# tkmct/halo2-aes

Hardware: AMD Instinct MI355X
Metric: AES-128 block witnesses/sec (higher is better)
Workload: dtype u8

## Files before the change

### halo2-aes_amd/_build.py

```python
from __future__ import annotations

import os
import shutil
import subprocess
from pathlib import Path

PKG = Path(__file__).resolve().parent
ROOT = PKG.parent
CSRC = PKG / "csrc"
LIB = PKG / "libaesw.so"
HOST_LIB = PKG / "libaesw_host.so"
INCLUDE = ROOT / "include"


def _newer(target: Path, sources) -> bool:
    if not target.exists():
        return False
    t = target.stat().st_mtime
    return all(Path(s).stat().st_mtime <= t for s in sources)


def _run(cmd, cwd=None):
    proc = subprocess.run(cmd, cwd=cwd, stdout=subprocess.PIPE, stderr=subprocess.STDOUT, text=True)
    if proc.returncode != 0:
# ... 6 lines not shown
        if cand and Path(cand).exists():
            return cand
    raise RuntimeError("hipcc not found")


def _build(target: Path, deps, command, force: bool, in_place: bool = False) -> Path:
    if not force and _newer(target, deps):
        return target
    import fcntl
    with open(PKG / ".build.lock", "w") as lock:
        fcntl.flock(lock, fcntl.LOCK_EX)
        try:
            if not force and _newer(target, deps):
                return target
            tmp = target if in_place else target.with_suffix(".so.tmp%d" % os.getpid())
            _run(command(tmp))
            os.replace(tmp, target)
        finally:
            fcntl.flock(lock, fcntl.LOCK_UN)
    return target


def build_host(force: bool = False) -> Path:
    host = PKG / "host"
    srcs = [host / "host_capi.cpp"]
    deps = srcs + [INCLUDE / "aesw.h", INCLUDE / "aesw_host.h", host / "halo2_lite.hpp", host / "aes_gadget.hpp", LIB]
    return _build(HOST_LIB, deps, lambda tmp: ["g++", "-O2", "-std=c++17", "-fPIC", "-shared", "-Wall", "-o", str(tmp)] + [str(s) for s in srcs] +
                  ["-L" + str(PKG), "-laesw", "-Wl,-rpath,$ORIGIN"], force)


PRODUCT_SOURCES = [CSRC / n for n in ("aesw_kernels.hip", "aesw_api.cpp", "aesw_keyring.cpp", "aesw_hostpath.cpp", "aesw_arena.cpp",
                                      "aesw_comm.cpp", "aesw_group.cpp", "aesw_circuits.cpp")]
PRODUCT_HEADERS = [CSRC / n for n in ("aesw_lane.h", "aesw_layout.h", "aesw_flush.h", "aesw_slabmap.h", "aesw_check.h", "aesw_check_dev.h", "aesw_internal.h", "aesw_ctx.h",
                                      "aesw_keyring.h", "aesw_options.h", "aesw_placement.h")] + \
    [INCLUDE / "aesw.h"]


def _hipcc_shared(sources, out, extra_flags=(), link=()):
    return [hipcc_path(), "--offload-arch=gfx950", "-O3", "-std=c++17", "-fPIC", "-shared", "-Wall", "-pthread"] + list(extra_flags) + \
        ["-o", str(out)] + [str(s) for s in sources] + list(link)


def build_product(force: bool = False, extra_flags=(), out: Path = LIB, extra_sources=()) -> Path:
    srcs = PRODUCT_SOURCES + [Path(s) for s in extra_sources]
    return _build(Path(out), srcs + PRODUCT_HEADERS, lambda tmp: _hipcc_shared(srcs, tmp, extra_flags), force)


SATELLITE_HEADERS = [CSRC / n for n in ("aesw_check_dev.h", "aesw_check.h", "aesw_layout.h", "aesw_slabmap.h", "aesw_internal.h", "aesw_ctx.h",
                                        "aesw_keyring.h", "aesw_options.h", "aesw_placement.h")] + [INCLUDE / "aesw.h"]
SATELLITES = {
    "circ": ([CSRC / "circ" / "aesw_circ_check.hip"], [CSRC / "aesw_circ_search.h"], INCLUDE / "aesw_circ.h"),
    "cols": ([CSRC / "cols" / "aesw_cols_check.hip"], [CSRC / "aesw_circ_search.h"], INCLUDE / "aesw_cols.h"),
    "vals": ([CSRC / "vals" / "aesw_vals_check.hip"], [CSRC / "aesw_vals_check.h"], INCLUDE / "aesw_vals.h"),
    "acc": ([CSRC / "acc" / "aesw_acc.hip"], [CSRC / "aesw_mult.h", CSRC / "aesw_mult_dev.h", CSRC / "aesw_run.h", INCLUDE / "aesw_mult.h"], INCLUDE / "aesw_acc.h"),
    "perm": ([CSRC / "perm" / "aesw_perm.hip"], [CSRC / "aesw_mult.h", CSRC / "aesw_perm.h", INCLUDE / "aesw_mult.h"], INCLUDE / "aesw_perm.h"),
    "vacc": ([CSRC / "vacc" / "aesw_vacc.hip"], [CSRC / "aesw_mult.h", CSRC / "aesw_mult_dev.h", CSRC / "aesw_run.h", CSRC / "aesw_vals_check.h", CSRC / "aesw_vacc.h",
              INCLUDE / "aesw_mult.h"],
             INCLUDE / "aesw_vacc.h"),
    "mult": ([CSRC / "mult" / "aesw_mult.hip"], [CSRC / "aesw_mult.h", CSRC / "aesw_mult_dev.h"], INCLUDE / "aesw_mult.h"),
}
CIRC_LIB, COLS_LIB, VALS_LIB, ACC_LIB, PERM_LIB, VACC_LIB, MULT_LIB = (PKG / ("libaesw_%s.so" % name) for name in SATELLITES)

FIELD_LIBRARIES = {
    "theta": ([CSRC / "theta" / "aesw_theta.hip"], [CSRC / "aesw_fr.h", CSRC / "aesw_theta.h", CSRC / "aesw_mult.h", INCLUDE / "aesw_mult.h"],
              INCLUDE / "aesw_theta.h"),
}
THETA_LIB = PKG / "libaesw_theta.so"
# ... 7 lines not shown
```

### halo2-aes_amd/api.py

```python
from __future__ import annotations

import ctypes as C
from collections import namedtuple
from pathlib import Path

import numpy as np

from . import constants as K

_PKG = Path(__file__).resolve().parent
LIB_PATH = _PKG / "libaesw.so"
HOST_LIB_PATH = _PKG / "libaesw_host.so"
COLS_LIB_PATH = _PKG / "libaesw_cols.so"
VALS_LIB_PATH = _PKG / "libaesw_vals.so"
MULT_LIB_PATH = _PKG / "libaesw_mult.so"
ACC_LIB_PATH = _PKG / "libaesw_acc.so"
VACC_LIB_PATH = _PKG / "libaesw_vacc.so"
PERM_LIB_PATH = _PKG / "libaesw_perm.so"
THETA_LIB_PATH = _PKG / "libaesw_theta.so"
CIRC_LIB_PATH = _PKG / "libaesw_circ.so"

STATUS = {
    0: "AESW_OK", 1: "AESW_ERR_INVALID_ARG", 2: "AESW_ERR_NO_DEVICE", 3: "AESW_ERR_HIP", 4: "AESW_ERR_NOMEM",
    5: "AESW_ERR_CAPACITY", 6: "AESW_ERR_NO_KEY", 7: "AESW_ERR_MISMATCH", 8: "AESW_ERR_UNSATISFIED", 9: "AESW_ERR_COMM",
# ... 601 lines not shown
        ct = torch.empty((n, 16), dtype=torch.uint8, device=dev) if want_ct else None
        key = None
        if key_slab:
            m = n if n_keys is None else n_keys
            key = KeyWitness(torch.empty(m * K.WORDS_ROWS, dtype=torch.uint8, device=dev),
                             *[torch.empty(m * key_column_stride(layout, c), dtype=torch.uint8, device=dev)
                               for c in range(3)], None)
        return Witness(cols[0], cols[1], cols[2], ct, key)

    def alloc_columns(self, n: int, layout: int = K.LAYOUT_PACKED, want_ct: bool = False, key_slab: bool = False, key_only: bool = False):
        torch = self._torch()
        cols = Columns()
        if key_only:
            key_slab = True
        self._check(self._lib.aesw_columns_alloc(self._h, n, layout, 2 if key_only else (1 if key_slab else 0), 1 if want_ct else 0, C.byref(cols)),
                    "aesw_columns_alloc")
        dev = self._dev()

        def view(ptr, nbytes):
            if not ptr or not nbytes:
                return torch.empty(0, dtype=torch.uint8, device=dev)
            return torch.as_tensor(_DevView(ptr, nbytes), device=dev)

        x, y, z = (view(getattr(cols, c), n * column_stride(layout, i) if not key_only else 0) for i, c in enumerate("xyz"))
        ct = view(cols.ct, n * 16).view(n, 16) if want_ct else None
        key = None
        if key_slab:
            key = KeyWitness(view(cols.key.w, n * K.WORDS_ROWS), *[view(getattr(cols.key, c), n * key_column_stride(layout, i))
                                                                   for i, c in enumerate(("kx", "ky", "kz"))], None)
        wit = ArenaWitness(x, y, z, ct, key)
        wit.columns = cols
        self._arenas[id(cols)] = cols
        self.last_arena = {"candidates": int(cols.candidates), "chosen": int(cols.chosen), "probe_us": float(cols.probe_us),
                           "fill_us": float(cols.fill_us), "bytes": int(cols.bytes)}
        return wit

    def free_columns(self, wit) -> None:
        cols = getattr(wit, "columns", None)
        if cols is None or self._arenas.pop(id(cols), None) is None:
            raise ValueError("not a witness of alloc_columns (or already freed)")
        wit.columns = None
        self._check(self._lib.aesw_columns_free(self._h, C.byref(cols)), "aesw_columns_free")

    def schedule_key(self, key, layout: int = K.LAYOUT_PACKED, key_slab: bool = True):
        torch = self._torch()
        key = self._u8(key, "key")
        if key.numel() != 16:
            raise ValueError("key must be uint8[16]")
        out = ks = None
        if key_slab:
            dev = self._dev()
            out = KeyWitness(torch.empty(K.WORDS_ROWS, dtype=torch.uint8, device=dev),
                             *[torch.empty(key_column_stride(layout, c), dtype=torch.uint8, device=dev) for c in range(3)],
                             None)
            ks = KeySlab(*[t.data_ptr() for t in out[:4]])
        rc = self._lib.aesw_schedule_key_device(self._h, key.data_ptr(), layout, _ptr(ks),
                                                self._stream())
        self._check(rc, "aesw_schedule_key_device")
        return out

    def encrypt_witness(self, pt, keys, layout: int = K.LAYOUT_PACKED, out: Witness | None = None,
                        want_ct: bool = False, key_slab: bool = False) -> Witness:
        pt = self._u8(pt, "pt")
        if pt.dim() != 2 or pt.shape[1] != 16:
            raise ValueError("pt must be [n,16]")
        n = pt.shape[0]
        if keys is None:
# ... 804 lines not shown
```

### halo2-aes_amd/csrc/aesw_api.cpp

```cpp
#include <hip/hip_runtime.h>

#include <cstdio>
#include <cstdlib>
#include <cstring>
#include <algorithm>
#include <mutex>
#include <new>
#include <string>
#include <vector>

#include "../../include/aesw.h"
#include "aesw_internal.h"
#include "aesw_check.h"

using namespace aesw;

#include "aesw_ctx.h"

namespace {

bool aligned16(const void *p) { return (reinterpret_cast<uintptr_t>(p) & 15u) == 0; }
bool aligned4(const void *p) { return (reinterpret_cast<uintptr_t>(p) & 3u) == 0; }
bool valid_layout(int l) { return aesw_valid_layout(l); }

// ... 84 lines not shown
    return AESW_OK;
}

int check_witness_impl(aesw_ctx *ctx, const uint8_t *d_pt, const uint8_t *d_keys, int per_block_keys, uint64_t n, int layout,
                       const uint8_t *d_x, const uint8_t *d_y, const uint8_t *d_z, const uint8_t *d_ct, const aesw_key_slab *ks,
                       aesw_check_report *d_report, void *stream, bool skip_shared_key) {
    static_assert(sizeof(aesw_check_report) == 7 * sizeof(uint64_t), "the kernels address the report as seven u64");
    if (!ctx || !d_report || (layout != AESW_LAYOUT_DENSE && layout != AESW_LAYOUT_PACKED)) return AESW_ERR_INVALID_ARG;
    if (per_block_keys && n && !d_keys) return AESW_ERR_INVALID_ARG;
    if (n && (!d_pt || !d_x || !d_y || !d_z || !ks || !ks->w || !ks->kx || !ks->ky || !ks->kz)) return AESW_ERR_INVALID_ARG;
    if (n && (!aligned4(d_pt) || !aligned4(d_x) || !aligned4(d_y) || !aligned4(d_z) || !aligned4(ks->w) || !aligned4(ks->kx) || !aligned4(ks->ky) ||
              !aligned4(ks->kz) || (reinterpret_cast<uintptr_t>(d_report) & 7u)))
        return AESW_ERR_INVALID_ARG;
    DeviceGuard g(ctx->device);
    if (!g.ok) return AESW_ERR_NO_DEVICE;
    const int li = layout == AESW_LAYOUT_DENSE ? 0 : 1;
    const CheckGeo cg = check_geo(layout);
    CheckParams p{};
    p.pt = d_pt; p.keys = d_keys; p.x = d_x; p.y = d_y; p.z = d_z; p.ct = d_ct;
    if (ks) set_key_slab(p, ks);
    p.table = ctx->d_chktab[li];
    p.tab768 = ctx->d_tables;
    p.report = reinterpret_cast<uint64_t *>(d_report);
    p.n = n;
    p.per_block_keys = per_block_keys ? 1u : 0u;
    p.skip_shared_key = skip_shared_key ? 1u : 0u;
    set_strides(p, slab_strides(layout));
    p.bi = cg.bi;
    p.img = (cg.bi + cg.ki + 15u) & ~15u;
    HIP_TRY(ctx, launch_check(p, reinterpret_cast<hipStream_t>(stream)));
    return AESW_OK;
}

namespace {

struct EncLaunch {
    const uint8_t *d_pt, *d_keys;
    int per_block_keys;
    uint64_t n;
    int layout;
    uint8_t *d_x, *d_y, *d_z, *d_ct;
    KeyOut ko;
    bool kemit;
};

bool validate_encrypt(const aesw_ctx *ctx, const uint8_t *d_pt, const uint8_t *d_keys, int per_block_keys, uint64_t n, int layout, uint8_t *d_x,
                     uint8_t *d_y, uint8_t *d_z, uint8_t *d_ct, const aesw_key_slab *ks, EncLaunch *L, int *status) {
    *status = AESW_ERR_INVALID_ARG;
    if (!ctx || !valid_layout(layout)) return false;
    if (!d_keys) {
        if (per_block_keys) return false;
        if (!ctx->keys.has_key()) { *status = AESW_ERR_NO_KEY; return false; }
    }
    *L = EncLaunch{d_pt, d_keys, per_block_keys, n, layout, d_x, d_y, d_z, d_ct, KeyOut{nullptr, nullptr, nullptr, nullptr}, false};
    *status = AESW_OK;
    if (n == 0) return false;
    *status = AESW_ERR_INVALID_ARG;
    const bool has_x = slab_strides(layout).x != 0;
    if (!d_pt || (has_x && !d_x) || !d_y || !d_z) return false;
    if ((has_x && !aligned16(d_x)) || !aligned16(d_y) || !aligned16(d_z) || !aligned4(d_pt) || (d_keys && !aligned4(d_keys)) ||
        (d_ct && !aligned4(d_ct)))
        return false;
    if (!key_out_of(ks, &L->ko)) return false;
    L->kemit = L->ko.w || L->ko.kx || L->ko.ky || L->ko.kz;
    if (!d_keys && L->kemit) return false;
    *status = AESW_OK;
    return true;
}

int enqueue_encrypt(aesw_ctx *ctx, const EncLaunch &L, hipStream_t s) {
    if (!L.per_block_keys && L.kemit) {
        KeyParams kp{L.d_keys, ctx->d_tables, L.ko, nullptr, 1, 0, 0};
        HIP_TRY(ctx, launch_key(kp, L.layout, ctx->xt, 1, ctx->opt.key_nt, 0u, s));
    }
    const int km = L.per_block_keys ? 0 : (L.d_keys ? 1 : 2);
    KeyRing::Access rd;
    if (km == 2) {
        const int rc = ctx->keys.begin_read(ctx, s, &rd);
        if (rc != AESW_OK) return rc;
    }
    EncParams p{L.d_pt, L.d_keys, reinterpret_cast<const uint32_t *>(rd.d), ctx->d_tables, ctx->d_ftab[L.layout], L.d_x, L.d_y, L.d_z, L.d_ct,
                L.per_block_keys ? L.ko : KeyOut{nullptr, nullptr, nullptr, nullptr}, L.n, 0, 0};
#ifdef AESW_TRACE
    p.trace = ctx->trace;
#endif
    HIP_TRY(ctx, launch_encrypt(p, L.layout, ctx->xt, km, L.per_block_keys && L.kemit, auto_waves(ctx, L.layout, L.per_block_keys != 0),
                                ctx->opt.nt, (uint32_t)ctx->opt.grid_cap, ctx->opt.xcd_remap, (uint32_t)ctx->opt.lds_pad, s));
    return km == 2 ? ctx->keys.end_read(ctx, rd) : AESW_OK;
}

template <class Issue>
int fork_join(aesw_ctx *ctx, hipStream_t s, uint32_t ns, uint32_t count, Issue &&issue) {
    if (!ctx->ev_fork) HIP_TRY(ctx, hipEventCreateWithFlags(&ctx->ev_fork, hipEventDisableTiming));
    for (uint32_t j = 0; j < ns; ++j) {
        if (!ctx->s_batch[j]) HIP_TRY(ctx, hipStreamCreateWithFlags(&ctx->s_batch[j], hipStreamNonBlocking));
        if (!ctx->ev_join[j]) HIP_TRY(ctx, hipEventCreateWithFlags(&ctx->ev_join[j], hipEventDisableTiming));
    }
    HIP_TRY(ctx, hipEventRecord(ctx->ev_fork, s));
    for (uint32_t j = 0; j < ns; ++j) HIP_TRY(ctx, hipStreamWaitEvent(ctx->s_batch[j], ctx->ev_fork, 0));
    int rc = AESW_OK;
    for (uint32_t i = 0; i < count && rc == AESW_OK; ++i) rc = issue(i, ctx->s_batch[i % ns]);
    for (uint32_t j = 0; j < ns; ++j) {
        const hipError_t e1 = hipEventRecord(ctx->ev_join[j], ctx->s_batch[j]);
        const hipError_t e2 = e1 == hipSuccess ? hipStreamWaitEvent(s, ctx->ev_join[j], 0) : e1;
        if (e2 != hipSuccess && rc == AESW_OK) rc = fail_hip(ctx, e2, "join of the batch streams");
    }
    return rc;
}

int encrypt_lone(aesw_ctx *ctx, const EncLaunch &L, hipStream_t s) {
    if (ctx->opt.split_small <= 1 || L.per_block_keys || L.kemit || L.n < ((uint64_t)1 << 15) || L.n > ((uint64_t)1 << 17)) return enqueue_encrypt(ctx, L, s);
    const uint32_t parts = (uint32_t)ctx->opt.split_small;
    const uint64_t per = ((L.n + parts - 1) / parts + 47) / 48 * 48;
    const uint32_t cnt = (uint32_t)((L.n + per - 1) / per);
    const SlabStrides st = slab_strides(L.layout);
    return fork_join(ctx, s, cnt, cnt, [&](uint32_t i, hipStream_t si) {
        const uint64_t lo = i * per;
        EncLaunch part = L;
        part.d_pt += lo * 16;
        part.n = L.n - lo < per ? L.n - lo : per;
// ... 395 lines not shown
```

### halo2-aes_amd/csrc/aesw_arena.cpp

```cpp
#include <hip/hip_runtime.h>

#include <algorithm>
#include <chrono>
#include <cstring>
#include <vector>

#include "../../include/aesw.h"
#include "aesw_ctx.h"
#include "aesw_internal.h"

using namespace aesw;

namespace {
bool valid_layout(int l) { return aesw_valid_layout(l); }
}

extern "C" {

namespace {

int vmm_build(aesw_ctx *ctx, size_t total, size_t chunk, void **out) {
    hipMemAllocationProp prop = {};
    prop.type = hipMemAllocationTypePinned;
    prop.location.type = hipMemLocationTypeDevice;
    prop.location.id = ctx->device;
    hipMemAccessDesc acc = {};
    acc.location = prop.location;
    acc.flags = hipMemAccessFlagsProtReadWrite;
    void *va = nullptr;
    HIP_TRY(ctx, hipMemAddressReserve(&va, total, 0, nullptr, 0));
    size_t mapped = 0;
    hipError_t e = hipSuccess;
    while (mapped < total && e == hipSuccess) {
        const size_t sz = total - mapped < chunk ? total - mapped : chunk;
        hipMemGenericAllocationHandle_t h;
        e = hipMemCreate(&h, sz, &prop, 0);
        if (e != hipSuccess) break;
        e = hipMemMap(reinterpret_cast<uint8_t *>(va) + mapped, sz, 0, h, 0);
        (void)hipMemRelease(h);
        if (e == hipSuccess) mapped += sz;
// ... 55 lines not shown
    DeviceGuard g(ctx->device);
    if (!g.ok) return AESW_ERR_NO_DEVICE;
    auto fill_out = [&](uint8_t *b) {
        auto at = [&](int i) -> uint8_t * { return size[i] ? b + off[i] : nullptr; };
        out->x = at(0); out->y = at(1); out->z = at(2); out->ct = at(3);
        out->key.w = at(4); out->key.kx = at(5); out->key.ky = at(6); out->key.kz = at(7);
    };
    int probe = ctx->opt.arena_probe < 0 ? (n >= ((uint64_t)1 << 16) ? 8 : 0) : ctx->opt.arena_probe;
    if (probe == 0) {
        uint8_t *raw = nullptr;
        HIP_TRY(ctx, hipMalloc(reinterpret_cast<void **>(&raw), end + align));
        out->base = raw;
        out->bytes = end + align;
        fill_out(raw + (align - reinterpret_cast<uintptr_t>(raw) % align) % align);
        return AESW_OK;
    }
    if (ctx->opt.arena_cache_on) {
        for (size_t i = ctx->arena_cache.size(); i-- > 0;) {
            aesw_ctx::ArenaRec &c = ctx->arena_cache[i];
            if (c.n == n && c.layout == layout && c.with_key_slab == with_key_slab && c.with_ct == (with_ct ? 1 : 0) && c.xcd == ctx->opt.xcd_remap) {
                *out = c.cols;
                out->candidates = 0;
                ctx->vmm_arenas.push_back(std::move(c));
                ctx->arena_cache.erase(ctx->arena_cache.begin() + (long)i);
                ++ctx->arena_cache_hits;
                return AESW_OK;
            }
        }
        size_t free_b = 0, total_b = 0;
        if (hipMemGetInfo(&free_b, &total_b) != hipSuccess) { (void)hipGetLastError(); free_b = 0; }
        if (free_b < 2 * end + ((size_t)16 << 30)) cache_trim(ctx, 0);
    }
    const auto t_search = std::chrono::steady_clock::now();
    auto over_budget = [&]() {
        if (ctx->opt.arena_probe_budget_ms <= 0) return false;
        return std::chrono::duration_cast<std::chrono::milliseconds>(std::chrono::steady_clock::now() - t_search).count() > ctx->opt.arena_probe_budget_ms;
    };
    using Range = aesw_ctx::ArenaRange;
    const size_t MiB2 = (size_t)2 << 20;
    auto round2m = [&](uint64_t v) { return (size_t)((v + MiB2 - 1) / MiB2 * MiB2); };
    auto build = [&](int kind, size_t bytes, Range *r) -> int {
        static const size_t chunk_of[4] = {(size_t)8 << 20, (size_t)2 << 20, (size_t)32 << 20, (size_t)4 << 20};
        if (kind % 5 == 0) {
            void *q = nullptr;
            HIP_TRY(ctx, hipMalloc(&q, bytes));
            *r = Range{q, bytes, false};
            return AESW_OK;
        }
        void *va = nullptr;
        const int rc = vmm_build(ctx, bytes, chunk_of[(kind % 5) - 1], &va);
        if (rc == AESW_OK) *r = Range{va, bytes, true};
        return rc;
    };
    aesw_ctx::ArenaRec rec{nullptr, {}};
    std::vector<Range> losers;
    hipEvent_t e0 = nullptr, e1 = nullptr, e2 = nullptr, e3 = nullptr;
    bool done = false;
    struct Cleanup {
        aesw_ctx::ArenaRec &rec; std::vector<Range> &losers; bool &done; hipEvent_t &a, &b, &d, &e;
        ~Cleanup() {
            for (auto &r : losers) { if (r.vmm) vmm_release(r.p, r.bytes); else (void)hipFree(r.p); }
            if (!done)
                for (auto &r : rec.ranges) { if (r.vmm) vmm_release(r.p, r.bytes); else (void)hipFree(r.p); }
            if (a) (void)hipEventDestroy(a);
            if (b) (void)hipEventDestroy(b);
            if (d) (void)hipEventDestroy(d);
            if (e) (void)hipEventDestroy(e);
        }
    } cleanup{rec, losers, done, e0, e1, e2, e3};
    HIP_TRY(ctx, hipEventCreate(&e3));
    HIP_TRY(ctx, hipEventCreate(&e0));
    HIP_TRY(ctx, hipEventCreate(&e1));
    HIP_TRY(ctx, hipEventCreate(&e2));
    ProbeParams pp = {};
    for (int c = 0; c < 7; ++c) pp.stride[c] = c < 3 && key_only ? 0 : st[c];
    pp.n = n;
    pp.xcd_mode = ctx->opt.xcd_remap;
    const int passes = n >= ((uint64_t)1 << 20) ? 2 : (int)std::min<uint64_t>(32, (((uint64_t)1 << 21) + n - 1) / n);
    const float accept = n >= ((uint64_t)1 << 18) ? 1.025f : 1.065f;
    uint32_t total_cands = 0;
    struct Placement {
        std::vector<Range> ranges;
        uint8_t *col[7] = {nullptr, nullptr, nullptr, nullptr, nullptr, nullptr, nullptr};
        uint8_t *ct = nullptr;
        float probe_us = 0.f, fill_us = 1.f;
        int rc = AESW_OK;
    };
    auto search = [&](int unit_mode) -> Placement {
        Placement pl;
        ProbeParams q = pp;
        for (int c = 0; c < 7; ++c) q.col[c] = nullptr;
        std::vector<std::vector<int>> units;
        if (unit_mode == 0) {
            units.push_back({0, 1, 2, 3, 4, 5, 6});
        } else {
            int order[7] = {0, 1, 2, 3, 4, 5, 6};
            std::sort(order, order + 7, [&](int a, int b) { return size[size_of7[a]] > size[size_of7[b]]; });
            for (int c : order)
                if (size[size_of7[c]]) units.push_back({c});
        }
        auto fail = [&](int rc) { for (auto &r : pl.ranges) losers.push_back(r); pl.ranges.clear(); pl.rc = rc; return pl; };
        auto hip = [&](hipError_t e, const char *what) { return e == hipSuccess ? AESW_OK : fail_hip(ctx, e, what); };
        for (size_t ui = 0; ui < units.size(); ++ui) {
            const std::vector<int> &cols = units[ui];
            size_t uoff[8], ubytes = 0;
            for (int c : cols) { uoff[c] = ubytes; ubytes += round2m(size[size_of7[c]]); }
            const bool with_ct_here = unit_mode == 0 && size[3];
            if (with_ct_here) { uoff[7] = ubytes; ubytes += round2m(size[3]); }
            if (!ubytes) continue;
            Range best{nullptr, 0, false};
            float best_probe = 0.f, best_fill = 1.f;
            float ref_fill = 0.f;
            for (int k = 0; k < probe; ++k) {
                if (best.p && over_budget()) break;
                if (best.p) {
                    size_t free_b = 0, total_b = 0;
                    if (hipMemGetInfo(&free_b, &total_b) != hipSuccess) { (void)hipGetLastError(); free_b = 0; }
                    if (free_b < ubytes + ((size_t)16 << 30)) break;
                }
                Range r{nullptr, 0, false};
                int rc = build(k + (int)ui, ubytes, &r);
                if (rc != AESW_OK) {
                    (void)hipGetLastError();
                    if (!best.p) return fail(rc);
                    break;
                }
                losers.push_back(r);
                ++total_cands;
                for (int c : cols) q.col[c] = size[size_of7[c]] ? reinterpret_cast<uint8_t *>(r.p) + uoff[c] : nullptr;
                rc = hip(launch_probe(q, false, nullptr), "probe launch");
                if (rc == AESW_OK) rc = hip(hipEventRecord(e0, nullptr), "hipEventRecord");
                for (int i = 0; i < passes && rc == AESW_OK; ++i) rc = hip(launch_probe(q, false, nullptr), "probe launch");
                if (rc == AESW_OK) rc = hip(hipEventRecord(e1, nullptr), "hipEventRecord");
                if (rc == AESW_OK) rc = hip(launch_probe(q, true, nullptr), "probe launch");
                if (rc == AESW_OK) rc = hip(hipEventRecord(e3, nullptr), "hipEventRecord");
                for (int i = 0; i < passes && rc == AESW_OK; ++i) rc = hip(launch_probe(q, true, nullptr), "probe launch");
                if (rc == AESW_OK) rc = hip(hipEventRecord(e2, nullptr), "hipEventRecord");
                if (rc == AESW_OK) rc = hip(hipEventSynchronize(e2), "hipEventSynchronize");
                float f = 0, l = 0;
                if (rc == AESW_OK) rc = hip(hipEventElapsedTime(&f, e0, e1), "hipEventElapsedTime");
                if (rc == AESW_OK) rc = hip(hipEventElapsedTime(&l, e3, e2), "hipEventElapsedTime");
                if (rc != AESW_OK) return fail(rc);
                {
                    double probed_bytes = 0;
                    for (int c = 0; c < 7; ++c) if (q.col[c]) probed_bytes += (double)n * q.stride[c];
                    if (probed_bytes >= 1e9) {
                        const double per_gb = (double)l * 1e3 / passes / (probed_bytes * 1e-9);
                        if (ctx->best_fill_us_per_gb == 0 || per_gb < ctx->best_fill_us_per_gb) ctx->best_fill_us_per_gb = per_gb;
                        const float floor_ms = (float)(ctx->best_fill_us_per_gb * probed_bytes * 1e-9 * passes * 1e-3);
                        if (l > 1.03f * floor_ms) l = 1.03f * floor_ms;
                    }
                }
                if (ref_fill == 0.f || l < ref_fill) ref_fill = l;
                const float ratio = f / ref_fill;
                if (!best.p || f < best_probe * passes * 1e-3f) { best = r; best_probe = f * 1e3f / passes; }
                best_fill = ref_fill * 1e3f / passes;
                if (ratio <= accept) break;
            }
            for (size_t i = 0; i < losers.size(); ++i)
                if (losers[i].p == best.p) { losers.erase(losers.begin() + (long)i); break; }
            pl.ranges.push_back(best);
            for (int c : cols) q.col[c] = size[size_of7[c]] ? reinterpret_cast<uint8_t *>(best.p) + uoff[c] : nullptr;
            if (with_ct_here) pl.ct = reinterpret_cast<uint8_t *>(best.p) + uoff[7];
            pl.probe_us = best_probe;
            pl.fill_us = best_fill;
        }
        if (size[3] && !pl.ct) {
            Range r{nullptr, 0, false};
            const int rc = build(1, round2m(size[3]), &r);
            if (rc != AESW_OK) return fail(rc);
            pl.ranges.push_back(r);
            pl.ct = reinterpret_cast<uint8_t *>(r.p);
        }
        for (int c = 0; c < 7; ++c) pl.col[c] = q.col[c];
        return pl;
    };
    Placement pl = search(ctx->opt.arena_unit == 1 ? 1 : 0);
    if (pl.rc != AESW_OK) return pl.rc;
    if (ctx->opt.arena_unit == 2 && n >= ((uint64_t)1 << 18) && pl.probe_us > accept * pl.fill_us && !over_budget()) {
        Placement alt = search(1);
        if (alt.rc == AESW_OK && alt.probe_us / alt.fill_us < pl.probe_us / pl.fill_us) std::swap(pl, alt);
        for (auto &r : alt.ranges) losers.push_back(r);
    }
    rec.ranges = pl.ranges;
    out->x = pl.col[0]; out->y = pl.col[1]; out->z = pl.col[2]; out->ct = pl.ct;
    out->key.w = pl.col[3]; out->key.kx = pl.col[4]; out->key.ky = pl.col[5]; out->key.kz = pl.col[6];
    out->base = reinterpret_cast<uint8_t *>(rec.ranges[0].p);
    for (auto &r : rec.ranges) out->bytes += r.bytes;
    out->candidates = total_cands;
    out->chosen = 0;
    out->probe_us = pl.probe_us;
    out->fill_us = pl.fill_us;
    rec.key = out->base;
    rec.n = n; rec.layout = layout; rec.with_key_slab = with_key_slab; rec.with_ct = with_ct ? 1 : 0; rec.xcd = ctx->opt.xcd_remap;
    rec.cols = *out;
    ctx->vmm_arenas.push_back(rec);
    done = true;
    return AESW_OK;
}

}

void aesw_arena_cache_trim(aesw_ctx *ctx, uint64_t keep_bytes) {
    DeviceGuard g(ctx->device);
    if (g.ok) cache_trim(ctx, keep_bytes);
}

extern "C" {

int aesw_columns_free(aesw_ctx *ctx, aesw_columns *cols) {
    if (!ctx || !cols) return AESW_ERR_INVALID_ARG;
    if (aesw_is_group(ctx)) return aesw_group_refuse(ctx, "aesw_columns_free");
    if (cols->base) {
        DeviceGuard g(ctx->device);
        if (!g.ok) return AESW_ERR_NO_DEVICE;
        bool vmm = false;
        for (size_t i = 0; i < ctx->vmm_arenas.size(); ++i)
            if (ctx->vmm_arenas[i].key == cols->base) {
                HIP_TRY(ctx, hipDeviceSynchronize());
                if (ctx->opt.arena_cache_on && ctx->vmm_arenas[i].cols.bytes <= ctx->opt.arena_cache_max_bytes()) {
                    ctx->vmm_arenas[i].stamp = ++ctx->arena_stamp;
                    ctx->arena_cache.push_back(std::move(ctx->vmm_arenas[i]));
                    ctx->vmm_arenas.erase(ctx->vmm_arenas.begin() + (long)i);
// ... 16 lines not shown
```

### halo2-aes_amd/csrc/aesw_ctx.h

```cpp
#pragma once
#include <hip/hip_runtime.h>

#include <cstdio>
#include <ctime>
#include <string>
#include <vector>

#include "../../include/aesw.h"
#include "aesw_keyring.h"
#include "aesw_options.h"

struct aesw_ctx {
    int device = -1;
    uint8_t *d_tables = nullptr;
    uint8_t *d_fr_lut = nullptr;
    uint32_t *d_ftab[3] = {nullptr, nullptr, nullptr};
    uint32_t *d_chktab[2] = {nullptr, nullptr};
    KeyRing keys;
    bool xt = false;
    AeswOptions opt;
    double best_fill_us_per_gb = 0;
    struct ArenaRange { void *p; size_t bytes; bool vmm; };
    struct ArenaRec {
        void *key;
// ... 62 lines not shown
    explicit DeviceGuard(int dev) {
        if (hipGetDevice(&prev) != hipSuccess) prev = -1;
        ok = hipSetDevice(dev) == hipSuccess;
    }
    ~DeviceGuard() {
        if (prev >= 0) (void)hipSetDevice(prev);
    }
};

void aesw_arena_cache_trim(aesw_ctx *ctx, uint64_t keep_bytes);

inline bool aligned_to(const void *p, uintptr_t a) { return (reinterpret_cast<uintptr_t>(p) & (a - 1)) == 0; }
inline bool key_slab_ok(const aesw_key_slab *ks) {
    return ks && ks->w && ks->kx && ks->ky && ks->kz && aligned_to(ks->w, 16) && aligned_to(ks->kx, 16) && aligned_to(ks->ky, 16) && aligned_to(ks->kz, 16);
}
inline uint64_t now_ns() {
    timespec ts;
    clock_gettime(CLOCK_MONOTONIC, &ts);
    return (uint64_t)ts.tv_sec * 1000000000ull + (uint64_t)ts.tv_nsec;
}

inline void merge_check_report(aesw_check_report &t, const aesw_check_report &r, uint64_t first_block, bool per_block_keys) {
    t.blocks += r.blocks; t.keys += r.keys;
    t.lookup_failures += r.lookup_failures; t.copy_failures += r.copy_failures;
    t.gate_failures += r.gate_failures; t.input_failures += r.input_failures;
    if (r.first == AESW_CHECK_NONE) return;
    const uint64_t unit = AESW_CHECK_UNIT(r.first) + ((!per_block_keys && AESW_CHECK_IS_KEY_SLAB(r.first)) ? 0 : first_block);
    const uint64_t f = unit << 20 | (r.first & 0xfffffu);
    if (f < t.first) t.first = f;
}

inline bool aesw_valid_layout(int l) { return l == AESW_LAYOUT_DENSE || l == AESW_LAYOUT_PACKED || l == AESW_LAYOUT_VALUES; }

namespace aesw { struct AssembleParams; }
AESW_INTERNAL int fill_assemble_params(aesw_ctx *ctx, uint32_t k, uint32_t n_sets, uint64_t n_blocks, int layout, const uint8_t *d_x,
                                       const uint8_t *d_y, const uint8_t *d_z, const aesw_key_slab *ks, aesw::AssembleParams *p);
AESW_INTERNAL int check_witness_impl(aesw_ctx *ctx, const uint8_t *d_pt, const uint8_t *d_keys, int per_block_keys, uint64_t n, int layout,
                                     const uint8_t *d_x, const uint8_t *d_y, const uint8_t *d_z, const uint8_t *d_ct, const aesw_key_slab *ks,
                                     aesw_check_report *d_report, void *stream, bool skip_shared_key);
AESW_INTERNAL int auto_copy_threads(const aesw_ctx *ctx);
```

### include/aesw.h

```cpp
#ifndef AESW_H
#define AESW_H

#include <stddef.h>
#include <stdint.h>

#ifdef __cplusplus
extern "C" {
#endif

#define AESW_VERSION 102

#define AESW_AES_ROWS 1360u
#define AESW_KEY_SCHEDULE_ROWS 1760u
#define AESW_KEY_ROWS 400u
#define AESW_WORDS_ROWS 96u
#define AESW_TABLE_ROWS 66561u
#define AESW_FR_BYTES 32u

enum aesw_status {
    AESW_OK = 0,
    AESW_ERR_INVALID_ARG = 1,
    AESW_ERR_NO_DEVICE = 2,
    AESW_ERR_HIP = 3,
    AESW_ERR_NOMEM = 4,
// ... 88 lines not shown
#define AESW_CHECK_KIND(f) (((f) >> 16) & 7u)
#define AESW_CHECK_INDEX(f) ((f) & 0xffffu)
int aesw_check_witness_device(aesw_ctx *ctx, const uint8_t *d_pt, const uint8_t *d_keys, int per_block_keys,
                              uint64_t n, int layout, const uint8_t *d_x, const uint8_t *d_y,
                              const uint8_t *d_z, const uint8_t *d_ct, const aesw_key_slab *d_key_slab,
                              aesw_check_report *d_report, void *stream);

int aesw_expand_fr_device(aesw_ctx *ctx, const uint8_t *d_cells, uint64_t n_cells, uint8_t *d_fr,
                          void *stream);

int aesw_assemble_advice_device(aesw_ctx *ctx, uint32_t k, uint32_t n_sets, uint64_t n_blocks,
                                int layout, const uint8_t *d_x, const uint8_t *d_y,
                                const uint8_t *d_z, const aesw_key_slab *d_key_slab, int as_fr,
                                uint8_t *d_out, void *stream);

int aesw_assemble_advice_circuits_device(aesw_ctx *ctx, uint32_t k, uint32_t n_sets, uint32_t n_circuits,
                                         const uint64_t *d_offsets, int layout, const uint8_t *d_x,
                                         const uint8_t *d_y, const uint8_t *d_z,
                                         const aesw_key_slab *d_key_slabs, int as_fr, uint8_t *d_out, void *stream);

typedef struct aesw_columns {
    uint8_t *base;
    uint64_t bytes;
    uint8_t *x;
    uint8_t *y;
    uint8_t *z;
    uint8_t *ct;
    aesw_key_slab key;
    uint32_t candidates;
    uint32_t chosen;
    float probe_us;
    float fill_us;
} aesw_columns;
int aesw_columns_alloc(aesw_ctx *ctx, uint64_t n, int layout, int with_key_slab, int with_ct,
                       aesw_columns *out);
int aesw_columns_free(aesw_ctx *ctx, aesw_columns *cols);

void *aesw_host_alloc(size_t bytes);
void aesw_host_free(void *p);
int aesw_encrypt_witness(aesw_ctx *ctx, const uint8_t *pt, const uint8_t *keys, int per_block_keys,
                         uint64_t n, int layout, uint8_t *x, uint8_t *y, uint8_t *z, uint8_t *ct,
                         const aesw_key_slab *key_slab);
typedef int (*aesw_chunk_fn)(void *user, uint64_t first_block, uint64_t n_blocks, const uint8_t *x,
                             const uint8_t *y, const uint8_t *z);
int aesw_encrypt_witness_stream(aesw_ctx *ctx, const uint8_t *pt, const uint8_t *keys,
                                int per_block_keys, uint64_t n, int layout, aesw_chunk_fn consume,
                                void *user);
typedef struct aesw_stream_stats {
    uint64_t chunks;
    uint64_t bytes_to_host;
    uint64_t kernel_ns;
    uint64_t d2h_ns;
    uint64_t consumer_ns;
    uint64_t wait_ns;
    uint64_t wall_ns;
} aesw_stream_stats;
int aesw_last_stream_stats(const aesw_ctx *ctx, aesw_stream_stats *out);
typedef int (*aesw_column_fn)(void *user, uint32_t column, const uint8_t *cells, uint64_t n_cells);
int aesw_assemble_advice_stream(aesw_ctx *ctx, uint32_t k, uint32_t n_sets, uint64_t n_blocks,
                                int layout, const uint8_t *d_x, const uint8_t *d_y,
                                const uint8_t *d_z, const aesw_key_slab *d_key_slab, int as_fr,
                                aesw_column_fn consume, void *user);
int aesw_assemble_advice_host(aesw_ctx *ctx, uint32_t k, uint32_t n_sets, uint64_t n_blocks,
                              int layout, const uint8_t *d_x, const uint8_t *d_y,
                              const uint8_t *d_z, const aesw_key_slab *d_key_slab, int as_fr,
                              uint8_t *out);
// ... 39 lines not shown
```

### rust/aesw-sys/src/lib.rs

```rust
#![allow(non_camel_case_types)]

use std::os::raw::{c_char, c_int, c_void};

pub const AESW_VERSION: c_int = 102;

pub const AESW_AES_ROWS: u32 = 1360;
pub const AESW_KEY_SCHEDULE_ROWS: u32 = 1760;
pub const AESW_KEY_ROWS: u32 = 400;
pub const AESW_WORDS_ROWS: u32 = 96;
pub const AESW_TABLE_ROWS: u32 = 66561;
pub const AESW_FR_BYTES: u32 = 32;
pub const AESW_BLOCK_COPIES: u32 = 1952;
pub const AESW_KEY_COPIES: u32 = 640;
pub const AESW_COMM_ID_BYTES: u32 = 128;

pub const AESW_OK: c_int = 0;
pub const AESW_ERR_INVALID_ARG: c_int = 1;
pub const AESW_ERR_NO_DEVICE: c_int = 2;
pub const AESW_ERR_HIP: c_int = 3;
pub const AESW_ERR_NOMEM: c_int = 4;
pub const AESW_ERR_CAPACITY: c_int = 5;
pub const AESW_ERR_NO_KEY: c_int = 6;
pub const AESW_ERR_MISMATCH: c_int = 7;
pub const AESW_ERR_UNSATISFIED: c_int = 8;
pub const AESW_ERR_COMM: c_int = 9;

pub const AESW_LAYOUT_DENSE: c_int = 0;
pub const AESW_LAYOUT_PACKED: c_int = 1;
pub const AESW_LAYOUT_VALUES: c_int = 2;

pub const AESW_COL_X: c_int = 0;
pub const AESW_COL_Y: c_int = 1;
pub const AESW_COL_Z: c_int = 2;

#[repr(C)]
pub struct aesw_ctx {
    _private: [u8; 0],
}

#[repr(C)]
pub struct aesw_comm {
    _private: [u8; 0],
}

#[repr(C)]
#[derive(Clone, Copy, Debug)]
pub struct aesw_key_slab {
    pub w: *mut u8,
    pub kx: *mut u8,
    pub ky: *mut u8,
    pub kz: *mut u8,
}

#[repr(C)]
#[derive(Clone, Copy, Debug, Default, PartialEq, Eq)]
pub struct aesw_copy_edge {
    pub dst_space: u8,
    pub dst_col: u8,
    pub dst_row: u16,
    pub src_space: u8,
    pub src_col: u8,
    pub src_row: u16,
// ... 368 lines not shown
```

Baseline: 1.784 billion.

## Probe arena placements with the real encrypt kernel and factor out search policy

The arena placement search now times candidate column placements by running the actual encrypt kernel (writing into the candidate columns from a scratch input buffer) instead of an emulated write-pattern probe. Acceptance and stopping logic moves into a separate ArenaSearchPolicy with a size-dependent fast threshold, and the per-column fallback search is seeded from the first placement. The aim is to choose physical memory placements that match the real kernel's access behaviour, so the witness kernel runs against better-placed columns. In exchange, allocation takes longer and needs an extra scratch buffer, and kernel timings are noisier to compare.

After: 1.785 billion, median of 3. About the same (+0.0%).

```diff
diff --git a/halo2-aes_amd/_build.py b/halo2-aes_amd/_build.py
--- a/halo2-aes_amd/_build.py
+++ b/halo2-aes_amd/_build.py
@@ -62,7 +62,7 @@
 PRODUCT_SOURCES = [CSRC / n for n in ("aesw_kernels.hip", "aesw_api.cpp", "aesw_keyring.cpp", "aesw_hostpath.cpp", "aesw_arena.cpp",
                                       "aesw_comm.cpp", "aesw_group.cpp", "aesw_circuits.cpp")]
 PRODUCT_HEADERS = [CSRC / n for n in ("aesw_lane.h", "aesw_layout.h", "aesw_flush.h", "aesw_slabmap.h", "aesw_check.h", "aesw_check_dev.h", "aesw_internal.h", "aesw_ctx.h",
-                                      "aesw_keyring.h", "aesw_options.h", "aesw_placement.h")] + \
+                                      "aesw_keyring.h", "aesw_options.h", "aesw_placement.h", "aesw_arena_policy.h")] + \
     [INCLUDE / "aesw.h"]
 
 
diff --git a/halo2-aes_amd/api.py b/halo2-aes_amd/api.py
--- a/halo2-aes_amd/api.py
+++ b/halo2-aes_amd/api.py
@@ -657,7 +657,8 @@
         wit.columns = cols
         self._arenas[id(cols)] = cols
         self.last_arena = {"candidates": int(cols.candidates), "chosen": int(cols.chosen), "probe_us": float(cols.probe_us),
-                           "fill_us": float(cols.fill_us), "bytes": int(cols.bytes)}
+                           "fill_us": float(cols.fill_us), "bytes": int(cols.bytes), "probe": "kernel" if cols.chosen == 1 else "emulated" if cols.probe_us > 0 else "none",
+                           "ratio": float(cols.probe_us) / float(cols.fill_us) if cols.fill_us > 0 else 0.0}
         return wit
 
     def free_columns(self, wit) -> None:
diff --git a/halo2-aes_amd/csrc/aesw_api.cpp b/halo2-aes_amd/csrc/aesw_api.cpp
--- a/halo2-aes_amd/csrc/aesw_api.cpp
+++ b/halo2-aes_amd/csrc/aesw_api.cpp
@@ -140,6 +140,15 @@
     return AESW_OK;
 }
 
+hipError_t launch_encrypt_of(const aesw_ctx *ctx, const EncParams &p0, int layout, int keymode, bool kemit, hipStream_t s) {
+    EncParams p = p0;
+#ifdef AESW_TRACE
+    p.trace = ctx->trace;
+#endif
+    return launch_encrypt(p, layout, ctx->xt, keymode, kemit, auto_waves(ctx, layout, keymode == 0), ctx->opt.nt, (uint32_t)ctx->opt.grid_cap,
+                          ctx->opt.xcd_remap, (uint32_t)ctx->opt.lds_pad, s);
+}
+
 namespace {
 
 struct EncLaunch {
@@ -189,11 +198,7 @@
     }
     EncParams p{L.d_pt, L.d_keys, reinterpret_cast<const uint32_t *>(rd.d), ctx->d_tables, ctx->d_ftab[L.layout], L.d_x, L.d_y, L.d_z, L.d_ct,
                 L.per_block_keys ? L.ko : KeyOut{nullptr, nullptr, nullptr, nullptr}, L.n, 0, 0};
-#ifdef AESW_TRACE
-    p.trace = ctx->trace;
-#endif
-    HIP_TRY(ctx, launch_encrypt(p, L.layout, ctx->xt, km, L.per_block_keys && L.kemit, auto_waves(ctx, L.layout, L.per_block_keys != 0),
-                                ctx->opt.nt, (uint32_t)ctx->opt.grid_cap, ctx->opt.xcd_remap, (uint32_t)ctx->opt.lds_pad, s));
+    HIP_TRY(ctx, launch_encrypt_of(ctx, p, L.layout, km, L.per_block_keys && L.kemit, s));
     return km == 2 ? ctx->keys.end_read(ctx, rd) : AESW_OK;
 }
 
diff --git a/halo2-aes_amd/csrc/aesw_arena.cpp b/halo2-aes_amd/csrc/aesw_arena.cpp
--- a/halo2-aes_amd/csrc/aesw_arena.cpp
+++ b/halo2-aes_amd/csrc/aesw_arena.cpp
@@ -6,6 +6,7 @@
 #include <vector>
 
 #include "../../include/aesw.h"
+#include "aesw_arena_policy.h"
 #include "aesw_ctx.h"
 #include "aesw_internal.h"
 
@@ -127,10 +128,7 @@
         if (free_b < 2 * end + ((size_t)16 << 30)) cache_trim(ctx, 0);
     }
     const auto t_search = std::chrono::steady_clock::now();
-    auto over_budget = [&]() {
-        if (ctx->opt.arena_probe_budget_ms <= 0) return false;
-        return std::chrono::duration_cast<std::chrono::milliseconds>(std::chrono::steady_clock::now() - t_search).count() > ctx->opt.arena_probe_budget_ms;
-    };
+    auto elapsed_ms = [&]() -> int64_t { return std::chrono::duration_cast<std::chrono::milliseconds>(std::chrono::steady_clock::now() - t_search).count(); };
     using Range = aesw_ctx::ArenaRange;
     const size_t MiB2 = (size_t)2 << 20;
     auto round2m = [&](uint64_t v) { return (size_t)((v + MiB2 - 1) / MiB2 * MiB2); };
@@ -147,13 +145,21 @@
         if (rc == AESW_OK) *r = Range{va, bytes, true};
         return rc;
     };
+#ifdef AESW_ARENA_PROBE_EMULATED
+    const bool by_kernel = false;
+#else
+    const bool by_kernel = !key_only && ctx->opt.arena_unit != 1;
+#endif
+    const bool pbk_probe = with_key_slab == 1;
     aesw_ctx::ArenaRec rec{nullptr, {}};
     std::vector<Range> losers;
     hipEvent_t e0 = nullptr, e1 = nullptr, e2 = nullptr, e3 = nullptr;
+    uint8_t *scratch = nullptr;
     bool done = false;
     struct Cleanup {
-        aesw_ctx::ArenaRec &rec; std::vector<Range> &losers; bool &done; hipEvent_t &a, &b, &d, &e;
+        aesw_ctx::ArenaRec &rec; std::vector<Range> &losers; bool &done; hipEvent_t &a, &b, &d, &e; uint8_t *&scratch;
         ~Cleanup() {
+            if (scratch) (void)hipFree(scratch);
             for (auto &r : losers) { if (r.vmm) vmm_release(r.p, r.bytes); else (void)hipFree(r.p); }
             if (!done)
                 for (auto &r : rec.ranges) { if (r.vmm) vmm_release(r.p, r.bytes); else (void)hipFree(r.p); }
@@ -162,7 +168,8 @@
             if (d) (void)hipEventDestroy(d);
             if (e) (void)hipEventDestroy(e);
         }
-    } cleanup{rec, losers, done, e0, e1, e2, e3};
+    } cleanup{rec, losers, done, e0, e1, e2, e3, scratch};
+    if (by_kernel) HIP_TRY(ctx, hipMalloc(reinterpret_cast<void **>(&scratch), n * 16 + (pbk_probe ? n * 16 : 16)));
     HIP_TRY(ctx, hipEventCreate(&e3));
     HIP_TRY(ctx, hipEventCreate(&e0));
     HIP_TRY(ctx, hipEventCreate(&e1));
@@ -181,10 +188,26 @@
         float probe_us = 0.f, fill_us = 1.f;
         int rc = AESW_OK;
     };
-    auto search = [&](int unit_mode) -> Placement {
+    auto launch_pattern = [&](const ProbeParams &q) -> hipError_t {
+        if (!by_kernel) return launch_probe(q, false, nullptr);
+        EncParams p{scratch, scratch + n * 16, nullptr, ctx->d_tables, ctx->d_ftab[layout], q.col[0], q.col[1], q.col[2], nullptr,
+                    pbk_probe ? KeyOut{q.col[3], q.col[4], q.col[5], q.col[6]} : KeyOut{nullptr, nullptr, nullptr, nullptr}, n, 0, 0};
+        return launch_encrypt_of(ctx, p, layout, pbk_probe ? 0 : 1, pbk_probe, nullptr);
+    };
+    bool want_columns = false;
+    auto search = [&](int unit_mode, const Placement *base) -> Placement {
         Placement pl;
         ProbeParams q = pp;
-        for (int c = 0; c < 7; ++c) q.col[c] = nullptr;
+        for (int c = 0; c < 7; ++c) q.col[c] = by_kernel && base ? base->col[c] : nullptr;
+        ArenaSearchPolicy policy;
+        policy.bar = accept;
+        policy.fast = n >= ((uint64_t)1 << 18) ? 1.0f : 1.04f;
+        policy.cap = probe;
+        policy.budget_ms = ctx->opt.arena_probe_budget_ms;
+        policy.columns_next = unit_mode == 0 && ctx->opt.arena_unit == 2 && n >= ((uint64_t)1 << 18);
+#ifdef AESW_ARENA_PROBE_EMULATED
+        policy.first_within_bar = true;
+#endif
         std::vector<std::vector<int>> units;
         if (unit_mode == 0) {
             units.push_back({0, 1, 2, 3, 4, 5, 6});
@@ -203,29 +226,25 @@
             const bool with_ct_here = unit_mode == 0 && size[3];
             if (with_ct_here) { uoff[7] = ubytes; ubytes += round2m(size[3]); }
             if (!ubytes) continue;
-            Range best{nullptr, 0, false};
-            float best_probe = 0.f, best_fill = 1.f;
-            float ref_fill = 0.f;
-            for (int k = 0; k < probe; ++k) {
-                if (best.p && over_budget()) break;
-                if (best.p) {
-                    size_t free_b = 0, total_b = 0;
-                    if (hipMemGetInfo(&free_b, &total_b) != hipSuccess) { (void)hipGetLastError(); free_b = 0; }
-                    if (free_b < ubytes + ((size_t)16 << 30)) break;
-                }
+            std::vector<Range> built;
+            policy.begin_unit();
+            ArenaSearchPolicy::Step step = ArenaSearchPolicy::ANOTHER;
+            for (int k = 0; step == ArenaSearchPolicy::ANOTHER; ++k) {
                 Range r{nullptr, 0, false};
                 int rc = build(k + (int)ui, ubytes, &r);
                 if (rc != AESW_OK) {
                     (void)hipGetLastError();
-                    if (!best.p) return fail(rc);
+                    if (built.empty()) return fail(rc);
+                    step = policy.closed(elapsed_ms());
                     break;
                 }
                 losers.push_back(r);
+                built.push_back(r);
                 ++total_cands;
                 for (int c : cols) q.col[c] = size[size_of7[c]] ? reinterpret_cast<uint8_t *>(r.p) + uoff[c] : nullptr;
-                rc = hip(launch_probe(q, false, nullptr), "probe launch");
+                rc = hip(launch_pattern(q), "probe launch");
                 if (rc == AESW_OK) rc = hip(hipEventRecord(e0, nullptr), "hipEventRecord");
-                for (int i = 0; i < passes && rc == AESW_OK; ++i) rc = hip(launch_probe(q, false, nullptr), "probe launch");
+                for (int i = 0; i < passes && rc == AESW_OK; ++i) rc = hip(launch_pattern(q), "probe launch");
                 if (rc == AESW_OK) rc = hip(hipEventRecord(e1, nullptr), "hipEventRecord");
                 if (rc == AESW_OK) rc = hip(launch_probe(q, true, nullptr), "probe launch");
                 if (rc == AESW_OK) rc = hip(hipEventRecord(e3, nullptr), "hipEventRecord");
@@ -236,22 +255,23 @@
                 if (rc == AESW_OK) rc = hip(hipEventElapsedTime(&f, e0, e1), "hipEventElapsedTime");
                 if (rc == AESW_OK) rc = hip(hipEventElapsedTime(&l, e3, e2), "hipEventElapsedTime");
                 if (rc != AESW_OK) return fail(rc);
+                float floor_ms = 0.f;
                 {
                     double probed_bytes = 0;
                     for (int c = 0; c < 7; ++c) if (q.col[c]) probed_bytes += (double)n * q.stride[c];
                     if (probed_bytes >= 1e9) {
                         const double per_gb = (double)l * 1e3 / passes / (probed_bytes * 1e-9);
                         if (ctx->best_fill_us_per_gb == 0 || per_gb < ctx->best_fill_us_per_gb) ctx->best_fill_us_per_gb = per_gb;
-                        const float floor_ms = (float)(ctx->best_fill_us_per_gb * probed_bytes * 1e-9 * passes * 1e-3);
-                        if (l > 1.03f * floor_ms) l = 1.03f * floor_ms;
+                        floor_ms = (float)(ctx->best_fill_us_per_gb * probed_bytes * 1e-9 * passes * 1e-3);
                     }
                 }
-                if (ref_fill == 0.f || l < ref_fill) ref_fill = l;
-                const float ratio = f / ref_fill;
-                if (!best.p || f < best_probe * passes * 1e-3f) { best = r; best_probe = f * 1e3f / passes; }
-                best_fill = ref_fill * 1e3f / passes;
-                if (ratio <= accept) break;
+                size_t free_b = 0, total_b = 0;
+                if (hipMemGetInfo(&free_b, &total_b) != hipSuccess) { (void)hipGetLastError(); free_b = 0; }
+                step = policy.timed(f, l, floor_ms, elapsed_ms(), free_b >= ubytes + ((size_t)16 << 30));
             }
+            const Range best = built[(size_t)policy.best()];
+            const float best_probe = policy.seen[(size_t)policy.best()].pattern * 1e3f / passes, best_fill = policy.yardstick() * 1e3f / passes;
+            if (step == ArenaSearchPolicy::PER_COLUMN) want_columns = true;
             for (size_t i = 0; i < losers.size(); ++i)
                 if (losers[i].p == best.p) { losers.erase(losers.begin() + (long)i); break; }
             pl.ranges.push_back(best);
@@ -270,10 +290,10 @@
         for (int c = 0; c < 7; ++c) pl.col[c] = q.col[c];
         return pl;
     };
-    Placement pl = search(ctx->opt.arena_unit == 1 ? 1 : 0);
+    Placement pl = search(ctx->opt.arena_unit == 1 ? 1 : 0, nullptr);
     if (pl.rc != AESW_OK) return pl.rc;
-    if (ctx->opt.arena_unit == 2 && n >= ((uint64_t)1 << 18) && pl.probe_us > accept * pl.fill_us && !over_budget()) {
-        Placement alt = search(1);
+    if (want_columns) {
+        Placement alt = search(1, &pl);
         if (alt.rc == AESW_OK && alt.probe_us / alt.fill_us < pl.probe_us / pl.fill_us) std::swap(pl, alt);
         for (auto &r : alt.ranges) losers.push_back(r);
     }
@@ -283,7 +303,7 @@
     out->base = reinterpret_cast<uint8_t *>(rec.ranges[0].p);
     for (auto &r : rec.ranges) out->bytes += r.bytes;
     out->candidates = total_cands;
-    out->chosen = 0;
+    out->chosen = by_kernel ? AESW_PROBE_KERNEL : AESW_PROBE_EMULATED;
     out->probe_us = pl.probe_us;
     out->fill_us = pl.fill_us;
     rec.key = out->base;
diff --git a/halo2-aes_amd/csrc/aesw_arena_policy.h b/halo2-aes_amd/csrc/aesw_arena_policy.h
--- /dev/null
+++ b/halo2-aes_amd/csrc/aesw_arena_policy.h
@@ -0,0 +1,44 @@
+#pragma once
+#include <cstddef>
+#include <cstdint>
+#include <vector>
+
+struct ArenaSearchPolicy {
+    enum Step { STOP = 0, ANOTHER = 1, PER_COLUMN = 2 };
+    struct Timed { float pattern, fill; };
+
+    float bar = 1.025f;
+    float fast = 1.0f;
+    int cap = 8;
+    int64_t budget_ms = 3000;
+    bool columns_next = false;
+    bool first_within_bar = false;
+
+    std::vector<Timed> seen;
+
+    void begin_unit() { seen.clear(); }
+    int best() const {
+        int b = -1;
+        for (size_t i = 0; i < seen.size(); ++i)
+            if (b < 0 || seen[i].pattern < seen[(size_t)b].pattern) b = (int)i;
+        return b;
+    }
+    float yardstick() const {
+        float y = 0.f;
+        for (const Timed &t : seen)
+            if (y == 0.f || t.fill < y) y = t.fill;
+        return y;
+    }
+    float ratio() const { return seen.empty() ? 0.f : seen[(size_t)best()].pattern / yardstick(); }
+    bool spent(int64_t elapsed_ms) const { return budget_ms > 0 && elapsed_ms > budget_ms; }
+
+    Step closed(int64_t elapsed_ms) const { return ratio() > bar && columns_next && !spent(elapsed_ms) ? PER_COLUMN : STOP; }
+    Step timed(float pattern, float fill, float floor, int64_t elapsed_ms, bool memory_left = true) {
+        if (floor > 0.f && fill > 1.03f * floor) fill = 1.03f * floor;
+        seen.push_back(Timed{pattern, fill});
+        const float r = ratio();
+        if (r <= fast || (first_within_bar && r <= bar)) return STOP;
+        if ((int)seen.size() < cap && !spent(elapsed_ms) && memory_left) return ANOTHER;
+        return closed(elapsed_ms);
+    }
+};
diff --git a/halo2-aes_amd/csrc/aesw_ctx.h b/halo2-aes_amd/csrc/aesw_ctx.h
--- a/halo2-aes_amd/csrc/aesw_ctx.h
+++ b/halo2-aes_amd/csrc/aesw_ctx.h
@@ -118,10 +118,11 @@
 
 inline bool aesw_valid_layout(int l) { return l == AESW_LAYOUT_DENSE || l == AESW_LAYOUT_PACKED || l == AESW_LAYOUT_VALUES; }
 
-namespace aesw { struct AssembleParams; }
+namespace aesw { struct AssembleParams; struct EncParams; }
 AESW_INTERNAL int fill_assemble_params(aesw_ctx *ctx, uint32_t k, uint32_t n_sets, uint64_t n_blocks, int layout, const uint8_t *d_x,
                                        const uint8_t *d_y, const uint8_t *d_z, const aesw_key_slab *ks, aesw::AssembleParams *p);
 AESW_INTERNAL int check_witness_impl(aesw_ctx *ctx, const uint8_t *d_pt, const uint8_t *d_keys, int per_block_keys, uint64_t n, int layout,
                                      const uint8_t *d_x, const uint8_t *d_y, const uint8_t *d_z, const uint8_t *d_ct, const aesw_key_slab *ks,
                                      aesw_check_report *d_report, void *stream, bool skip_shared_key);
+AESW_INTERNAL hipError_t launch_encrypt_of(const aesw_ctx *ctx, const aesw::EncParams &p, int layout, int keymode, bool kemit, hipStream_t s);
 AESW_INTERNAL int auto_copy_threads(const aesw_ctx *ctx);
diff --git a/include/aesw.h b/include/aesw.h
--- a/include/aesw.h
+++ b/include/aesw.h
@@ -144,6 +144,8 @@
     float probe_us;
     float fill_us;
 } aesw_columns;
+#define AESW_PROBE_EMULATED 0u
+#define AESW_PROBE_KERNEL 1u
 int aesw_columns_alloc(aesw_ctx *ctx, uint64_t n, int layout, int with_key_slab, int with_ct,
                        aesw_columns *out);
 int aesw_columns_free(aesw_ctx *ctx, aesw_columns *cols);
diff --git a/rust/aesw-sys/src/lib.rs b/rust/aesw-sys/src/lib.rs
--- a/rust/aesw-sys/src/lib.rs
+++ b/rust/aesw-sys/src/lib.rs
@@ -28,6 +28,9 @@
 pub const AESW_LAYOUT_DENSE: c_int = 0;
 pub const AESW_LAYOUT_PACKED: c_int = 1;
 pub const AESW_LAYOUT_VALUES: c_int = 2;
+
+pub const AESW_PROBE_EMULATED: u32 = 0;
+pub const AESW_PROBE_KERNEL: u32 = 1;
 
 pub const AESW_COL_X: c_int = 0;
 pub const AESW_COL_Y: c_int = 1;
```
